# vshiv18/khoice

Measured on AMD Instinct MI355X. Metric: distinct k-mers/sec (k=31, canonical), higher is better.
Workload: dtype u64

## Files before the change

khoice_amd/csrc/kh_engine.cpp:

```cpp
#include <hip/hip_runtime.h>

#include <algorithm>
#include <atomic>
#include <thread>
#include <chrono>
#include <cmath>
#include <memory>
#include <cstdarg>
#include <cstdio>
#include <cstdlib>
#include <cstring>
#include <map>
#include <mutex>
#include <string>
#include <vector>

#include "../../include/khoice_hip.h"
#include "kh_engine.h"
#include "kh_launch.h"
#include "kh_skm_rec.h"

static thread_local std::string g_last_error;

int kh_fail(int code, const char* fmt, ...) {
// ... 1789 lines not shown
    HIPCHK(hipMemcpyAsync(s->dev<u8>(off.ginfo), h_up, up_bytes, hipMemcpyHostToDevice, st));
    c->prof_end();

    KhSkmJob& job = s->job;
    job.seg_tag = by_group ? s->dev<const u8>(off.tags) : nullptr;
    job.segs = s->dev<const KhSeg>(off.segs);
    job.tiles = s->dev<const KhTile>(off.tiles);
    job.reg1 = s->d_reg1.as<uint4>();
    job.reg2 = s->d_reg2.as<uint4>();
    job.cur1 = s->dev<u32>(off.cur1);
    job.cur2 = s->dev<u32>(off.cur2);
    job.inst = s->dev<unsigned long long>(off.inst);
    job.dup = s->dev<unsigned long long>(off.dup);
    job.ginfo = s->dev<const u32>(off.ginfo);
    job.hist = s->dev<unsigned long long>(0);
    job.ctl = s->dev<u32>(off.ctl);
    job.claim = s->dev<u32>(off.claim);
    job.tile_pos = tile_pos;
    job.k = k; job.m = g.m; job.w = g.w; job.nmax = g.nmax;
    job.nslots = g.nslots; job.S = g.S; job.nb1 = g.nb1; job.cap1 = g.cap1; job.cap2 = g.cap2;
    job.nbins = L->nbins; job.abase = L->abase; job.reps = reps; job.nops = by_group ? (u32)ngroups : (u32)nseq;
    job.spill_rec = s->d_spill.as<uint4>();
    job.spill_slot = reinterpret_cast<u32*>(s->d_spill.as<u8>() + (size_t)spill_cap * rec_bytes);
    job.big_list = reinterpret_cast<u32*>(s->d_spill.as<u8>() + (size_t)spill_cap * (rec_bytes + 4));
    job.spill_cap = spill_cap;
    job.big_cap = SkmRun::big_cap;
#ifdef KH_STAMPS
    const u64 nst = std::max<u64>(ntiles, g.nslots);
    TMP_ALLOC(s->d_stamps, c, 128 * nst);
    HIPCHK(hipMemsetAsync(s->d_stamps.b->p, 0, 128 * nst, st));
    kh_debug_set_stamps_skm(s->d_stamps.as<u64>());
#endif
    c->prof_begin(KC_SKM_SCATTER);
    wd.scatter(job, ntiles, st);
    c->prof_end();
#ifdef KH_STAMPS
    report_stamps(c, "skm_scatter (second sub-tile: codes / hashes / minima / slots+count / - / append / barrier / -)", s->d_stamps.b, ntiles);
    HIPCHK(hipMemsetAsync(s->d_stamps.b->p, 0, 128 * nst, st));
    kh_debug_set_stamps_skm(nullptr);
#endif
    c->prof_begin(KC_SKM_REGROUP);
    wd.regroup(job, st);
    c->prof_end();
#ifdef KH_STAMPS
    kh_debug_set_stamps_skm(s->d_stamps.as<u64>());
#ifdef KH_STAMPS_WG
    kh_debug_set_stamps_skm2(s->d_stamps.as<u64>());
#endif
#endif
    s->staged = true;
    return KH_OK;
}
static int exp1_skm(kh_ctx* c, const Exp1In& in, uint64_t* within_hist, uint64_t* across_hist, uint64_t* distinct_per_seq,
                    bool* done, bool by_group = false) {
    *done = false;
    SkmRun s(c);
    KHCHK(skm_prepare(c, in.nseq, in.seqs, in.lens, in.on_device, in.group_of, in.ngroups, in.k, by_group, 0, 0, &s));
    if (!s.staged) return KH_OK;
    const TagLayout& L = s.L;
    const SkmGeometry& g = s.g;
    const KhSkmJob& job = s.job;
    hipStream_t st = c->st;
    KHCHK(timed_launch(c, KC_SKM_UNION, [&] { g.wd->unite(job, in.cs, g.ugrid, st); }));
#if defined(KH_STAMPS) && defined(KH_STAMPS_WG)
    dump_wg_ends(c, s.d_stamps.b, g.ugrid);
    kh_debug_set_stamps_skm(nullptr);
    kh_debug_set_stamps_skm2(nullptr);
#elif defined(KH_STAMPS)
    report_stamps(c, "skm_union (scan barrier / owner / expand / insert / barrier / read-out / barrier / flush)", s.d_stamps.b, g.nslots);
    kh_debug_set_stamps_skm(nullptr);
#endif
    if (getenv("KHOICE_SKM_DEBUG")) {
        std::vector<u32> h1(g.nb1), h2(g.nslots);
        HIPCHK(hipMemcpy2DAsync(h1.data(), 4, job.cur1, 4 * (size_t)KH_SKM_CUR1_STRIDE, 4, g.nb1, hipMemcpyDeviceToHost, st));
        HIPCHK(hipMemcpyAsync(h2.data(), job.cur2, 4 * (size_t)g.nslots, hipMemcpyDeviceToHost, st));
        u32 hc[KH_SKM_CTL_WORDS];
        HIPCHK(hipMemcpyAsync(hc, job.ctl, sizeof hc, hipMemcpyDeviceToHost, st));
        HIPCHK(hipStreamSynchronize(st));
        u64 t1 = 0, t2 = 0;
        u32 m1 = 0, m2 = 0;
        for (u32 v : h1) { t1 += v; m1 = std::max(m1, v); }
        for (u32 v : h2) { t2 += v; m2 = std::max(m2, v); }
        fprintf(stderr, "[skm] k=%d m=%d w=%u nmax=%u positions=%llu records=%llu (%.2f k-mers each) nb1=%u S=%u nslots=%u | "
                        "coarse: mean %.0f max %u cap %u | slot: mean %.1f max %u cap %u | tiles %u x %u | expanded: %u k-mers | errors %u spilled %u overfull slots %u multi-subset slots %u\n",
                in.k, g.m, g.w, g.nmax, (unsigned long long)g.positions, (unsigned long long)t1, (double)g.positions / std::max<u64>(1, t1),
                g.nb1, g.S, g.nslots, (double)t1 / g.nb1, m1, g.cap1, (double)t2 / g.nslots, m2, g.cap2, s.ntiles, job.tile_pos,
                hc[KH_SKM_CTL_EXPANDED], hc[KH_SKM_CTL_ERR], hc[KH_SKM_CTL_SPILLED], hc[KH_SKM_CTL_LISTED], g.two ? 0u : hc[KH_SKM_CTL_MULTI]);
    }
    bool declines = false;
    KHCHK(s.settle(0, [&](u32 nbig) {
        c->stat.big_slots += nbig;
        return timed_launch(c, KC_SKM_BIG, [&] { g.wd->big(job, in.cs, nbig, st); });
    }, &declines));
    if (declines) return KH_OK;
    c->stat.skm_records += s.h_ctl()[KH_SKM_CTL_RECORDS];
    if (!L.by_group) {
        c->stat.bases += s.bases;
        c->stat.builds += L.nseq;
        u64 isum = 0, dsum = 0;
        s.per_text([&](int t, u64 inst, u64 d) {
            isum += inst;
            dsum += d;
            if (distinct_per_seq) distinct_per_seq[t] = d;
        });
        c->stat.kmers += isum;
        c->stat.distinct += dsum;
        c->stat.setop_in += dsum;
    }
    c->stat.setops++;
    std::vector<u64> bins(L.nbins, 0);
    L.add_bins(bins, s.h_hist(), job.reps);
    L.fold(c, bins, within_hist, across_hist, in.hist_len);
    *done = true;
    return KH_OK;
}
static bool skm_exchange_k(int k) { return k >= KH_SKM_MIN_K && k <= KH_SKM_MAX_K; }

static bool skm_exchange_geometry(int k, uint64_t positions_max, int nparts, u32 fan, u64* nslots, double* per_kmer_out,
                                  double eff_parts = 0.0 ) {
    const int m = skm_minimizer_len(k);
    const u32 w = (u32)(k - m + 1);
    const double per_kmer = skm_per_kmer(w);
    const double clump = skm_clump(w, std::max<u32>(1, fan));
    auto region = [&](double mean) { return mean * per_kmer * skm_region_slack(clump, mean) + 128.0; };
    if (eff_parts <= 0.0) eff_parts = (double)nparts;
    double mean = std::min(2600.0 / (0.55 * eff_parts), (1024.0 - 128.0) / (1.7 * per_kmer));
    while (mean > 64.0 && region(mean) > 1008.0) mean *= 0.95;
    if (const char* e = getenv("KHOICE_SKM_EXCHANGE_MEAN")) mean = std::max(16.0, atof(e));
    u64 ns = std::max<u64>((u64)nparts, (u64)((double)std::max<u64>(1, positions_max) / mean) + 1);
    ns = std::min<u64>(ns, (u64)KH_SKM2_MAX_COARSE * KH_SKM_MAX_FINE);
    if (region((double)positions_max / (double)ns) > 1024.0) return false;
    *nslots = ns;
    *per_kmer_out = per_kmer;
    return true;
}
extern "C" int kh_skm_exchange_plan(kh_ctx* c, int k, uint64_t positions_max, uint32_t fan_max, int nparts, uint32_t* nslots,
                                    uint32_t* slots_per_part, uint64_t* part_cap) {
    if (!c || !nslots || !slots_per_part || !part_cap || nparts < 1) return kh_fail(KH_E_ARG, "kh_skm_exchange_plan: bad argument");
    if (!skm_exchange_k(k)) return kh_fail(KH_E_ARG, "the exchange form takes k = %d .. %d", KH_SKM_MIN_K, KH_SKM_MAX_K);
    u64 ns = 0;
    double per_kmer = 0;
    if (!skm_exchange_geometry(k, positions_max, nparts, fan_max, &ns, &per_kmer))
        return kh_fail(KH_E_CAPACITY, "too many k-mers per rank for the exchange form (%llu positions)", (unsigned long long)positions_max);
    *nslots = (u32)ns;
    *slots_per_part = (u32)((ns + nparts - 1) / nparts);
    *part_cap = skm_part_cap(positions_max, per_kmer, nparts);
    return KH_OK;
}

struct SkmPackLocal {
    std::vector<u64> inst;
    u64 dup[32] = {};
    Tmp spill;
    u32 spill_n = 0;
    bool done = false;
};
static int skm_pack_impl(kh_ctx* c, int nseq, const uint8_t* const* seqs, const uint64_t* lens, int on_device,
                         const int* tag_of, int k, uint32_t nslots, int nparts, uint64_t part_cap, void* rec_out,
                         uint32_t* mask_out, uint32_t* count_out, uint32_t* off_out, uint64_t* part_n, SkmPackLocal* loc) {
    if (loc) loc->done = false;
    if (!c || nseq < 0 || (nseq && (!seqs || !lens || !tag_of)) || nparts < 1 || !nslots || !rec_out || !mask_out || !count_out ||
        !off_out || !part_n)
        return kh_fail(KH_E_ARG, "kh_skm_pack: bad argument");
    if (!skm_exchange_k(k)) return kh_fail(KH_E_ARG, "the exchange form takes k = %d .. %d", KH_SKM_MIN_K, KH_SKM_MAX_K);
    int ntags = 0;
    for (int i = 0; i < nseq; ++i) {
        if (tag_of[i] < 0 || tag_of[i] >= 32) return kh_fail(KH_E_ARG, "kh_skm_pack: tag %d outside 0..31", tag_of[i]);
        ntags = std::max(ntags, tag_of[i] + 1);
    }
    HIPCHK(hipSetDevice(c->dev));
// ... 1839 lines not shown
```

khoice_amd/csrc/kh_launch.h:

```cpp
#pragma once
#include <hip/hip_runtime.h>
#include "kh_common.h"

struct KhSeg {
    const u8* seq;
    u64 len;
    u64 npos;
    u64 thist_base;
    u32 nbuckets;
    u32 bucket_base;
    u32 tile_base;
    u32 ntiles;
    u32 nb_virtual;
    u32 b_first;
};
struct KhTile { u32 seg; u32 tile_in_seg; };

struct KhBucketWork {
    u64 lo;
    u64 out_base;
    u32 n;
    u32 nb;
    u32 b;
    u32 gb;
};

struct KhSetView {
    const void* keys;
    const u32* counts;
    u64 n;
    u32 uniform;
    u32 pad;
};

struct KhBoundsJob {
    const KhSetView* sets;
    u64* bounds;
    u64* zero;
    u64 zero_words;
    u32 nsets, nranges;
};

constexpr int KH_SETOP_BATCH = 16;
struct KhSetopJob {
    const KhSetView* sets;
    const u64* bounds;
    void* out_keys;
    u32* out_counts;
    u64* desc;
    u32* ctl;
    unsigned long long* hist;
    u32 nsets;
    u32 nslots;
    u32 slot0, nranges;
};
struct KhSetopBatch { KhSetopJob job[KH_SETOP_BATCH]; };

struct KhGrid {
    u16* off;
    unsigned long long* distinct;
    u32 S;
    u32 nb;
};
constexpr int KH_TAG_MAX_OPS = 64;
constexpr int KH_TAG_MAX_BINS = 255;
struct KhTagJob {
    const void* keys;
    const u64* bstart;
    const u16* off;
    const u32* ginfo;
    unsigned long long* hist;
    u32* ctl;
    u32 nb, S, nops, nbins, abase, ngroups, reps;
    u32 nbv;
    u32 binmul;
    void* out_keys;
    u32* out_counts;
    u64* desc;
    unsigned long long* out_n;
};

#ifndef KH_TUNE_SKM_STAGE
#define KH_TUNE_SKM_STAGE 2048
#endif
constexpr u32 KH_SKM_STAGE = KH_TUNE_SKM_STAGE;
constexpr u32 KH_SKM_MAX_COARSE = 256;
constexpr u32 KH_SKM_MAX_FINE = 512;
constexpr int KH_SKM_MIN_K = 17, KH_SKM_MAX_K = 32;
#ifndef KH_TUNE_SKM_CUR1_STRIDE
#define KH_TUNE_SKM_CUR1_STRIDE 1088
#endif
constexpr u32 KH_SKM_CUR1_STRIDE = KH_TUNE_SKM_CUR1_STRIDE;
enum : u32 {
    KH_SKM_CTL_ERR = 0,
    KH_SKM_CTL_FULLEST = 1,
    KH_SKM_CTL_RECORDS = 2,
    KH_SKM_CTL_EXPANDED = 3,
    KH_SKM_CTL_SPILLED = 5,
    KH_SKM_CTL_LISTED = 6,
    KH_SKM_CTL_MULTI = 7,
    KH_SKM_CTL_WORDS = 8,
};
enum : u32 {
    KH_SKM_XCTL_ERR = 0,
    KH_SKM_XCTL_FULLEST = 1,
    KH_SKM_XCTL_CURSORS = 16,
};
struct KhSkmJob {
    const KhSeg* segs;
    const KhTile* tiles;
    const u8* seg_tag;
    uint4* reg1;
    uint4* reg2;
    u32* cur1;
    u32* cur2;
    unsigned long long* inst;
    unsigned long long* dup;
    const u32* ginfo;
    unsigned long long* hist;
    u32* ctl;
    u32* claim;
    u32 tile_pos;
    int k, m;
    u32 w;
    u32 nmax;
    u32 nslots, S, nb1, cap1, cap2;
    u32 nbins, abase, reps, nops;
    uint4* spill_rec;
    u32* spill_slot;
    u32* big_list;
    u32 spill_cap, big_cap;
};
struct KhSkmCrossJob {
    unsigned long long* bins;
    u32 pmlo, pmhi;
    u32 ngenomes;
    u32 nbins, reps;
    u32 nlisted;
};
struct KhSkmPivotJob {
    KhSkmCrossJob cj;
    u32 pinfo[KH_TAG_MAX_OPS];
};
constexpr int KH_SKM2_MAX_K = 63;
constexpr u32 KH_SKM2_MAX_COARSE = 512;
constexpr u32 KH_SKM2_MAX_FINE = 1024;
struct KhSkmWidth {
    u32 rec_bytes;
    u32 max_coarse, max_fine;
    u32 max_cap2;
    u32 table;
    u32 union_per_cu, cross_per_cu;
    u32 pivot_per_cu;
    u32 cross_round;
    bool (*supports_w)(u32 w);
    void (*scatter)(const KhSkmJob& job, u32 ntiles, hipStream_t st);
    void (*regroup)(const KhSkmJob& job, hipStream_t st);
    void (*unite)(const KhSkmJob& job, u32 cs, u32 grid, hipStream_t st);
    void (*big)(const KhSkmJob& job, u32 cs, u32 nbig, hipStream_t st);
    void (*cross)(const KhSkmJob& job, const KhSkmCrossJob& cj, u32 grid, hipStream_t st);
    void (*pivot)(const KhSkmJob& job, const KhSkmPivotJob& pj, u32 grid, hipStream_t st);
};
const KhSkmWidth& kh_skm_width1();
const KhSkmWidth& kh_skm_width2();
inline const KhSkmWidth& kh_skm_width(bool two) { return two ? kh_skm_width2() : kh_skm_width1(); }
struct KhSkmPackJob {
    const uint4* reg2;
    const u32* cur2;
    uint4* out_rec;
    u32* out_mask;
    u32* part_cursor;
    u32* slot_count;
    u32* slot_off;
    u32* ctl;
    unsigned long long* dup;
    u64 part_cap;
    u32 cap2, nslots, spp;
    u32 nsub;
};
struct KhSkmCompactJob {
// ... 175 lines not shown
```

khoice_amd/csrc/kh_skm.hip:

```cpp
#include <hip/hip_runtime.h>

#include "kh_device.h"
#include "kh_launch.h"

#ifdef KH_STAMPS
__device__ u64* g_skm_stamps = nullptr;
void kh_debug_set_stamps_skm(u64* p) { (void)hipMemcpyToSymbol(HIP_SYMBOL(g_skm_stamps), &p, sizeof p); }
#define SKM_STAMP(idx)                                                                     \
    do {                                                                                   \
        __builtin_amdgcn_sched_barrier(0);                                                 \
        if (threadIdx.x == 0 && g_skm_stamps)                                              \
            g_skm_stamps[((u64)blockIdx.y * gridDim.x + blockIdx.x) * 16 + (idx)] = __builtin_amdgcn_s_memtime(); \
        __builtin_amdgcn_sched_barrier(0);                                                 \
    } while (0)
#else
#define SKM_STAMP(idx) do {} while (0)
#endif

#ifdef KH_MARKS
#define SKM_MARK(name) asm volatile("; ===== MARK " name ::: "memory")
#else
#define SKM_MARK(name) do {} while (0)
#endif
#ifndef KH_TUNE_SKM_SCATTER_PREFETCH
// ... 266 lines not shown
using SkmUnion = SkmUnionGeo<1024, 4096>;
static_assert(SkmUnion::TABLE == 4096, "the slot geometry and its measurements (skm_plan) are the 4096-entry table's");

__device__ __forceinline__ u32 key_hash2(u32 lo, u32 hi) { return (lo ^ hi) * 0x9E3779B1u; }

struct Skm1Consts {
    u32 kml, kmh;
    u32 fsh;
    u32 tsh;
    u32 tsh_sub;
    bool tsh_high;
    __device__ __forceinline__ explicit Skm1Consts(const int k)
        : kml((u32)kh_mask(2 * k)), kmh((u32)(kh_mask(2 * k) >> 32)), fsh(64u - 2u * (u32)k), tsh(2u * (u32)k - 2u),
          tsh_sub(tsh >= 32u ? tsh - 32u : tsh), tsh_high(tsh >= 32u) {}
};
template <int E, class F>
__device__ __forceinline__ void skm1_expand(const uint4 r0, const u32 first, const Skm1Consts& kc, F&& f) {
    const u64 clo = ((u64)r0.y << 32) | r0.x, chi = ((u64)r0.w << 32) | r0.z;
    const u32 sh = 2u * first;
    const u64 lo = sh ? (clo >> sh) | (chi << (64u - sh)) : clo, hi = chi >> sh;
    const u32 xl = (u32)lo & kc.kml, xh = (u32)(lo >> 32) & kc.kmh;
    const u64 fw = kh_revpairs64(((u64)xh << 32) | xl) >> kc.fsh;
    u32 fl = (u32)fw, fh = (u32)(fw >> 32), rl = ~xl & kc.kml, rh = ~xh & kc.kmh;
    const u32 t = (u32)((lo >> kc.tsh) | (hi << (64u - kc.tsh)));
    const u32 tc = ~t;
#pragma unroll
    for (int e = 0; e < E; ++e) {
        if (e) {
            fh = __builtin_amdgcn_alignbit(fh, fl, 30) & kc.kmh;
            fl = ((fl << 2) | ((t >> (2 * e)) & 3u)) & kc.kml;
            rl = __builtin_amdgcn_alignbit(rh, rl, 2);
            rh >>= 2;
            if (kc.tsh_high) rh |= ((tc >> (2 * e)) & 3u) << kc.tsh_sub; else rl |= ((tc >> (2 * e)) & 3u) << kc.tsh_sub;
        }
        const bool fwd = fh < rh || (fh == rh && fl < rl);
        f((u32)e, fwd ? fl : rl, fwd ? fh : rh);
    }
}
struct SkmClaim1 {
    unsigned long long* tkey;
    u32 okey_off;
    unsigned long long empty, K;
    __device__ __forceinline__ u32 operator()(const bool second, const u32 S) const {
        const unsigned long long o2 = atomicCAS(tkey + (second ? okey_off : 0u) + S, empty, K);
        return o2 == empty ? SKM_FRESH : (o2 == K ? SKM_SAME_KEY : SKM_OTHER_KEY);
    }
};

#if defined(KH_STAMPS) && defined(KH_STAMPS_WG)
#define SKM_USTAMP(idx) do {} while (0)
#define SKM_WGSTAMP(idx)                                                                   \
    do {                                                                                   \
        __builtin_amdgcn_sched_barrier(0);                                                 \
        if (threadIdx.x == 0 && g_skm_stamps) {                                            \
            u64* const sp_ = g_skm_stamps + (u64)blockIdx.x * 16;                          \
            sp_[(idx)] = __builtin_amdgcn_s_memtime();                                     \
            sp_[(idx) + 3] = wall_clock64();                                               \
            if ((idx) == 0) {                                                              \
                sp_[1] = __builtin_amdgcn_s_getreg(4 | (31 << 11));                        \
                sp_[2] = __builtin_amdgcn_s_getreg(20 | (31 << 11));                       \
            }                                                                              \
        }                                                                                  \
        __builtin_amdgcn_sched_barrier(0);                                                 \
    } while (0)
#elif defined(KH_STAMPS)
#define SKM_WGSTAMP(idx) do {} while (0)
#define SKM_USTAMP(idx)                                                                    \
    do {                                                                                   \
        __builtin_amdgcn_sched_barrier(0);                                                 \
        if (threadIdx.x == 0 && g_skm_stamps) g_skm_stamps[(u64)slot * 16 + (idx)] = __builtin_amdgcn_s_memtime(); \
        __builtin_amdgcn_sched_barrier(0);                                                 \
    } while (0)
#else
#define SKM_USTAMP(idx) do {} while (0)
#define SKM_WGSTAMP(idx) do {} while (0)
#endif

#ifndef KH_TUNE_SKM_UNION_LEAN
#define KH_TUNE_SKM_UNION_LEAN 1
#endif
#ifndef KH_TUNE_SKM_UNION_KT
#define KH_TUNE_SKM_UNION_KT 1
#endif
template <u32 NT, u32 T, int KT>
__global__ __launch_bounds__(NT, 8) void k_skm_union(const KhSkmJob jb, u32 cs, u32 first_claimed) {
    extern __shared__ __attribute__((aligned(16))) u8 lds_raw[];
    using G = SkmUnionGeo<NT, T>;
    constexpr u32 T2 = G::T2, NW = NT / 64;
    constexpr u32 T2SH = 25;
    constexpr int E = (int)SKM_UE;
    constexpr u64 EMPTY = ~0ull;
    u8* p = lds_raw;
    unsigned long long* tkey = reinterpret_cast<unsigned long long*>(p);   p += (size_t)T * 8;
    u32* tmlo = reinterpret_cast<u32*>(p);                                 p += (size_t)T * 4;
    u32* tmhi = reinterpret_cast<u32*>(p);                                 p += (size_t)T * 4;
    unsigned long long* okey = reinterpret_cast<unsigned long long*>(p);   p += (size_t)T2 * 8;
    u32* omlo = reinterpret_cast<u32*>(p);                                 p += (size_t)T2 * 4;
    u32* omhi = reinterpret_cast<u32*>(p);                                 p += (size_t)T2 * 4;
    uint4* gtab = reinterpret_cast<uint4*>(p);                             p += 1024;
    u32* scratch = reinterpret_cast<u32*>(p);                              p += 128;
    u32* dupc = reinterpret_cast<u32*>(p);                                 p += 256;
    u32* hstripe = reinterpret_cast<u32*>(p);                              p += (size_t)SKM_HSTRIPE_WORDS * 4;
    u16* owner = reinterpret_cast<u16*>(p);                                p += (size_t)G::MAXCH * 2;
    u32* rmask = reinterpret_cast<u32*>(p);
    uint4* stage = reinterpret_cast<uint4*>(tkey);
    u32* dd = reinterpret_cast<u32*>(tkey) + T;
    const u32 tid0 = threadIdx.x, wid = __builtin_amdgcn_readfirstlane(tid0 >> 6);
    u32 tid = tid0, lane = lane_id();
    const u32 nbins = jb.nbins, cap2 = jb.cap2, nslots = jb.nslots;
    const int k = KT ? KT : jb.k;
    const u32 sshift = nbins <= 72u ? 2u : (nbins <= 144u ? 1u : 0u), smask = (1u << sshift) - 1u;
    auto clear_keys = [&]() {
        uint4* k4 = reinterpret_cast<uint4*>(tkey);
        for (u32 i = tid; i < T / 2; i += NT) k4[i] = make_uint4(0xffffffffu, 0xffffffffu, 0xffffffffu, 0xffffffffu);
    };
#if !(defined(KH_ABLATE) && KH_ABLATE == 3)
    constexpr bool MASKS_SELF_CLEAN = true;
#else
    constexpr bool MASKS_SELF_CLEAN = false;
#endif
    auto zero_masks = [&]() {
        for (u32 i = tid; i < T / 2; i += NT) reinterpret_cast<uint4*>(tmlo)[i] = make_uint4(0u, 0u, 0u, 0u);
        if (tid < T2) { omlo[tid] = 0u; omhi[tid] = 0u; }
    };
    auto clear_masks = [&]() {
        if (!MASKS_SELF_CLEAN) zero_masks();
        unsigned long long e0 = EMPTY;
        asm volatile("" : "+v"(e0));
        if (tid < T2) okey[tid] = e0;
    };
    typedef const u32 __attribute__((address_space(4))) * ConstU32;
    const ConstU32 counts = (ConstU32)(unsigned long long)jb.cur2;
    const u32 fit = cap2 < G::MAXREC ? cap2 : G::MAXREC;
    auto count_of = [&](u32 sl) -> u32 {
        const u32 n = sl < nslots ? counts[sl] : 0u;
        return n <= fit ? n : 0u;
    };
    SKM_MARK("init");
    if (MASKS_SELF_CLEAN) zero_masks();
    if (tid < (u32)KH_TAG_MAX_OPS) {
        const u32 g = jb.ginfo[tid], g0 = g & 0xffu, gn = (g >> 8) & 0xffu;
        const u64 gm = gn ? (gn >= 64u ? ~0ull : ((1ull << gn) - 1ull)) << g0 : 0ull;
        gtab[tid] = make_uint4((u32)gm, (u32)(gm >> 32), (g >> 16) << sshift, 0u);
        dupc[tid] = 0;
    }
    if (tid < SKM_HSTRIPE_WORDS) hstripe[tid] = 0;
    if (tid == 0) { scratch[0] = 0; scratch[1] = ~0u; }
    const u32 kml = (u32)kh_mask(2 * k), kmh = (u32)(kh_mask(2 * k) >> 32);
    const u32 fsh = 64u - 2u * (u32)k;
    const u32 tsh = 2u * (u32)k - 2u;
    const bool tsh_high = tsh >= 32u;
    const u32 tsh_sub = tsh_high ? tsh - 32u : tsh;
    auto eval_mask = [&](u32 mlo, u32 mhi) -> bool {
        const u32 lsel = lane & smask;
        u32 ng = 0;
        do {
            const u32 first = mlo ? (u32)__builtin_ctz(mlo) : 32u + (u32)__builtin_ctz(mhi);
            const uint4 g = gtab[first];
            u32 c = (u32)__popc(mlo & g.x) + (u32)__popc(mhi & g.y);
            c = c < cs ? c : cs;
            atomicAdd(&hstripe[g.z + (c << sshift) + lsel], 1u);
            const u32 keep_hi = mlo ? ~0u : mhi - 1u;
            mlo &= ~g.x & (mlo - 1u);
            mhi &= ~g.y & keep_hi;
            ++ng;
        } while (mlo | mhi);
        if (ng == 1u) return true;
        atomicAdd(&hstripe[((jb.abase + (ng < cs ? ng : cs)) << sshift) + lsel], 1u);
        return false;
    };
    u32 st_full = 0, st_exp = 0;
    SkmSlotFeed feed(gridDim.x, nslots, first_claimed);
    u32 slot = blockIdx.x, slot_next = slot + gridDim.x;
    u32 nrec = count_of(slot);
    u32 nrec_next = count_of(slot_next);
    uint4 rr = tid < nrec ? (jb.reg2 + (u64)slot * cap2)[tid] : make_uint4(0, 0, 0, 0);
    SKM_WGSTAMP(0);
    while (slot < nslots) {
        tid = tid0;
        asm volatile("" : "+v"(tid));
        lane = tid & (KH_WAVE - 1u);
        const uint4* __restrict__ reg = jb.reg2 + (u64)slot * cap2;
        if (!nrec && counts[slot] > fit) {
            if (tid0 == 0) {
                const u32 at = atomicAdd(jb.ctl + KH_SKM_CTL_LISTED, 1u);
                if (at < jb.big_cap) jb.big_list[at] = slot;
            }
        }
        u32 nj = 0;
        const u32 tg = SkmRec1::tag(rr.w);
        const u32 rx = rr.x, ry = rr.y, rz = rr.z, rw = rr.w;
        {
            u32 z = 0;
            asm volatile("" : "+v"(z));
            for (u32 i = tid; i < T / 4; i += NT) reinterpret_cast<uint4*>(dd)[i] = make_uint4(z, z, z, z);
        }
        if (tid < nrec) {
            nj = SkmRec1::n(rr.w);
            stage[tid] = rr;
            rmask[tid] = 1u << (tg & 31u);
        }
        SKM_USTAMP(0);
        __syncthreads();
        SKM_USTAMP(1);
        const u32 slot_after = feed.take(scratch + 1);
        const u32 nrec_after = count_of(slot_after);
        const bool draw = feed.wants();
        SKM_MARK("dedup");
        if (__builtin_amdgcn_ballot_w64(nj != 0)) {
            u32 h = rx * 0x9E3779B1u ^ ry * 0x85EBCA77u ^ rz * 0xC2B2AE3Du ^ SkmRec1::content_hash_word(rw) * 0x27D4EB2Fu;
            h ^= h >> 15;
            h *= 0x2C1B3C6Du;
            u32 hp = (u32)(((u64)h * T) >> 32);
            const u32 nch = (nj + (u32)E - 1u) / (u32)E;
            bool pend = nj != 0, won = false;
            while (__builtin_amdgcn_ballot_w64(pend)) {
                if (pend) {
                    const u32 old = atomicCAS(&dd[hp], 0u, tid + 1u);
                    if (old == 0u) {
                        won = true;
                        pend = false;
                    } else {
                        const uint4 o = stage[old - 1u];
                        if (o.x == rx && o.y == ry && o.z == rz && SkmRec1::same_content(o.w, rw)) {
                            const u32 bit = 1u << (tg & 31u);
                            const u32 was = atomicOr(&rmask[old - 1u], bit);
                            if (was & bit) {
                                atomicAdd(&dupc[tg], nj);
                                rmask[tid] = 0u;
                            }
                            pend = false;
                        } else {
                            hp = (hp + 1u) & (T - 1u);
                        }
                    }
                }
            }
            const u32 mine = won ? (nch | (nj << 16)) : 0u;
            const u32 incl = wave_scan_add(mine);
            u32 wbase = 0;
            if (lane == KH_WAVE - 1 && incl) wbase = atomicAdd(&scratch[0], incl);
            wbase = (u32)__builtin_amdgcn_readlane((int)wbase, KH_WAVE - 1);
            if (won) {
                const u32 cstart = (wbase + incl - mine) & 0xffffu;
                if (cstart + nch <= G::MAXCH) {
#pragma unroll
                    for (u32 cc = 0; cc < (1u << SKM_OB); ++cc)
                        if (cc < nch) owner[cstart + cc] = (u16)((tid << SKM_OB) | cc);
                }
            }
        }
        SKM_MARK("dedup_end");
        SKM_USTAMP(2);
        __syncthreads();
        const u32 sc0 = scratch[0];
        if ((sc0 & 0xffffu) > G::MAXCH) {
            if (tid < nrec && rmask[tid] == 0u) {
                const u32 w = stage[tid].w;
                atomicSub(&dupc[SkmRec1::tag(w)], SkmRec1::n(w));
            }
            __syncthreads();
        }
        rr = tid < nrec_next ? (jb.reg2 + (u64)slot_next * cap2)[tid] : make_uint4(0, 0, 0, 0);
        clear_keys();
        clear_masks();
        u32 C = sc0 & 0xffffu, N = sc0 >> 16;
        SKM_USTAMP(3);
        SKM_MARK("after_scan");
        st_full = N > st_full ? N : st_full;
        st_exp += N;
        if (C > G::MAXCH) {
            if (tid == 0) {
                if (jb.big_list) {
                    const u32 at = atomicAdd(jb.ctl + KH_SKM_CTL_LISTED, 1u);
                    if (at < jb.big_cap) jb.big_list[at] = slot;
                } else atomicOr(jb.ctl, KH_ERR_CAPACITY);
            }
            C = 0;
            N = 0;
        }
#if defined(KH_ABLATE) && KH_ABLATE == 1
        C = 0; N = 0;
#endif
        __syncthreads();
        if (tid == 0) scratch[0] = 0;
        SKM_MARK("owner_done");
        SKM_USTAMP(4);
        const u32 R0 = (N + T - 1) / T;
        auto slot_body = [&](auto multi_) __attribute__((always_inline)) {
            constexpr bool MULTI = decltype(multi_)::value;
            const u32 R = MULTI ? R0 : 1u;
            const u32 ctid = tid;
            for (u32 q = 0; q < R; ++q) {
                if (q) { clear_keys(); clear_masks(); __syncthreads(); }
                unsigned long long emptyv = EMPTY;
                asm volatile("" : "+v"(emptyv));
                u32 made[SKM_PASSES][E / 2];
#pragma unroll
                for (u32 ps = 0; ps < SKM_PASSES; ++ps)
#pragma unroll
                    for (int e = 0; e < E / 2; ++e) made[ps][e] = 0u;
                u32 ones = 0;
#pragma unroll
                for (u32 pass = 0; pass < SKM_PASSES; ++pass) {
                    if (pass * NT >= C) break;
                    const u32 c = pass * NT + ctid;
                    u64 kreg[E];
                    u32 slot_[E], act = 0, bits = 0, half = 0;
#pragma unroll
                    for (int e = 0; e < E; ++e) { kreg[e] = EMPTY; slot_[e] = 0; }
                    if (c < C) {
                        const u32 o = owner[c], ri = o >> SKM_OB, first = (o & ((1u << SKM_OB) - 1u)) * (u32)E;
                        const uint4 r0 = reg[ri];
                        bits = rmask[ri];
                        half = SkmRec1::half(r0.w);
                        const u32 left = SkmRec1::n(r0.w) - first;
                        const u32 cnt = left < (u32)E ? left : (u32)E;
                        const u64 clo = ((u64)r0.y << 32) | r0.x, chi = ((u64)r0.w << 32) | r0.z;
                        const u32 sh = 2u * first;
                        const u64 lo = sh ? (clo >> sh) | (chi << (64u - sh)) : clo, hi = chi >> sh;
                        const u32 xl = (u32)lo & kml, xh = (u32)(lo >> 32) & kmh;
                        const u64 fw = kh_revpairs64(((u64)xh << 32) | xl) >> fsh;
                        u32 fl = (u32)fw, fh = (u32)(fw >> 32), rl = ~xl & kml, rh = ~xh & kmh;
                        const u32 t = (u32)((lo >> tsh) | (hi << (64u - tsh)));
                        const u32 tc = ~t;
#pragma unroll
                        for (int e = 0; e < E; ++e) {
                            if (e) {
                                fh = __builtin_amdgcn_alignbit(fh, fl, 30) & kmh;
                                fl = ((fl << 2) | ((t >> (2 * e)) & 3u)) & kml;
                                rl = __builtin_amdgcn_alignbit(rh, rl, 2);
                                rh >>= 2;
                                if (tsh_high) rh |= ((tc >> (2 * e)) & 3u) << tsh_sub; else rl |= ((tc >> (2 * e)) & 3u) << tsh_sub;
                            }
                            const bool fwd = fh < rh || (fh == rh && fl < rl);
                            const u32 cl = fwd ? fl : rl, ch = fwd ? fh : rh;
                            const u32 h = key_hash2(cl, ch);
                            kreg[e] = ((u64)ch << 32) | cl;
                            slot_[e] = (u32)(((u64)h * T) >> 32);
                            if (R != 1 && (u32)e < cnt && (((h >> 4) & 0xffffu) * R) >> 16 == q) act |= 1u << e;
                        }
                        if (R == 1) act = (1u << cnt) - 1u;
                    }
#if defined(KH_ABLATE) && KH_ABLATE == 2
                    if (kreg[0] != 0x1234567ull) act = 0;
#endif
                    SKM_MARK("expanded");
                    if (!__builtin_amdgcn_ballot_w64(act != 0)) continue;
                    u32* const mp = half ? tmhi : tmlo;
                    u32 was[E];
#pragma unroll
                    for (int e = 0; e < E; ++e) was[e] = 0u;
                    u32 mk = 0;
                    for (u32 round = 0; round < (u32)KH_TUNE_SKM_FULL_ROUNDS && __builtin_amdgcn_ballot_w64(act != 0); ++round) {
                        unsigned long long old[E];
#pragma unroll
                        for (int e = 0; e < E; ++e)
                            old[e] = (act & (1u << e)) ? atomicCAS(&tkey[slot_[e]], emptyv, (unsigned long long)kreg[e]) : 0ull;
#pragma unroll
                        for (int e = 0; e < E; ++e) {
                            if (act & (1u << e)) {
                                const bool fresh = old[e] == emptyv;
                                if (fresh || old[e] == kreg[e]) {
                                    was[e] = atomicOr(mp + slot_[e], bits);
                                    act &= ~(1u << e);
                                    if (fresh) mk |= 1u << e;
                                } else {
                                    slot_[e] = (slot_[e] + 1u) & (T - 1u);
                                }
                            }
                        }
                    }
                    SKM_USTAMP(9);
                    SKM_MARK("rounds_done");
                    u32 f16[E];
#pragma unroll
                    for (int e = 0; e < E; ++e) f16[e] = (mk >> e) & 1u ? (0x8000u | slot_[e]) : 0u;
                    while (__builtin_amdgcn_ballot_w64(act != 0)) {
                        const bool have_one = act != 0;
                        const u32 es = have_one ? (u32)__builtin_ctz(act) : 0u;
                        u64 K = 0;
#pragma unroll
                        for (int e = 0; e < E; ++e)
                            if (es == (u32)e) K = kreg[e];
                        const u32 H = key_hash2((u32)K, (u32)(K >> 32));
                        u32 S = ((H ^ (H >> 15)) * 0x85EBCA77u) >> T2SH, probes = 0, level = 1;
                        bool mine = have_one;
                        u32 where = 0;
                        while (__builtin_amdgcn_ballot_w64(mine)) {
                            if (mine) {
                                unsigned long long* kp = level == 1 ? okey : tkey;
                                const unsigned long long o2 = atomicCAS(&kp[S], emptyv, (unsigned long long)K);
                                if (o2 == emptyv || o2 == K) {
                                    u32* mp2 = level == 1 ? (half ? omhi : omlo) : mp;
                                    u32 d = atomicOr(mp2 + S, bits) & bits;
                                    while (d) { atomicAdd(&dupc[half * 32u + (u32)__builtin_ctz(d)], 1u); d &= d - 1u; }
                                    if (o2 == emptyv) where = 0x8000u | (level == 1 ? 0x4000u : 0u) | S;
                                    mine = false;
                                } else {
                                    ++probes;
                                    if (level == 1 && probes >= 8u) {
                                        level = 2; probes = 0;
                                        S = (u32)(((u64)H * T) >> 32) + (u32)KH_TUNE_SKM_FULL_ROUNDS;
                                        S = S & (T - 1u);
                                    } else if (level == 2 && probes >= T) {
                                        atomicOr(jb.ctl, KH_ERR_CAPACITY);
                                        mine = false;
                                    } else {
                                        S = level == 1 ? ((S + 1u) & (T2 - 1u)) : ((S + 1u) & (T - 1u));
                                    }
                                }
                            }
                        }
                        if (have_one) {
                            act &= ~(1u << es);
#pragma unroll
                            for (int e = 0; e < E; ++e)
                                if (es == (u32)e) f16[e] = where;
                        }
                    }
                    SKM_MARK("serial_done");
#pragma unroll
                    for (int e = 0; e < E / 2; ++e) made[pass][e] = f16[2 * e] | (f16[2 * e + 1] << 16);
                    {
                        u32 d = 0;
#pragma unroll
                        for (int e = 0; e < E; ++e) d |= was[e] & bits;
                        if (d) {
#pragma unroll
                            for (int e = 0; e < E; ++e) {
                                u32 de = was[e] & bits;
                                while (de) { atomicAdd(&dupc[half * 32u + (u32)__builtin_ctz(de)], 1u); de &= de - 1u; }
                            }
                        }
                    }
                }
                SKM_MARK("insert_done");
                SKM_USTAMP(5);
                if (draw && q == 0 && tid0 == NT - KH_WAVE) feed.draw(jb.claim, scratch + 1);
                __syncthreads();
                SKM_USTAMP(6);
#pragma unroll
                for (u32 pass = 0; pass < SKM_PASSES; ++pass) {
                    u32 any = 0;
#pragma unroll
                    for (int e = 0; e < E / 2; ++e) any |= made[pass][e];
#if defined(KH_ABLATE) && KH_ABLATE == 3
                    if (any != 0x7654321u) any = 0;
#endif
                    if (!__builtin_amdgcn_ballot_w64(any != 0)) continue;
#pragma unroll
                    for (int e = 0; e < E; ++e) {
                        const u32 f = (made[pass][e >> 1] >> (16 * (e & 1))) & 0xffffu;
                        if (f & 0x8000u) {
                            const u32 at = f & 0x3fffu;
                            const bool second = f & 0x4000u;
                            u32 mlo, mhi;
                            if (MASKS_SELF_CLEAN) {
                                mlo = atomicExch((second ? omlo : tmlo) + at, 0u);
                                mhi = atomicExch((second ? omhi : tmhi) + at, 0u);
                            } else {
                                mlo = (second ? omlo : tmlo)[at];
                                mhi = (second ? omhi : tmhi)[at];
                            }
                            if (eval_mask(mlo, mhi)) ++ones;
                        }
                    }
                }
                if (__builtin_amdgcn_ballot_w64(ones != 0)) {
                    ones = wave_scan_add(ones);
                    if (lane == KH_WAVE - 1) atomicAdd(&hstripe[(jb.abase + 1u) << sshift], ones);
                }
                SKM_MARK("readout_done");
                SKM_USTAMP(7);
                if (q + 1 < R) __syncthreads();
            }
        };
        if (KH_TUNE_SKM_UNION_LEAN && R0 == 1u) {
            slot_body(std::false_type{});
        } else if (__builtin_expect(R0 != 0u, 0)) {
            if (R0 > 1u && tid0 == 0) atomicAdd(jb.ctl + KH_SKM_CTL_MULTI, 1u);
            slot_body(std::true_type{});
        }
        SKM_USTAMP(8);
        if (draw && R0 == 0 && tid0 == NT - KH_WAVE) feed.draw(jb.claim, scratch + 1);
        nrec = nrec_next;
        nrec_next = nrec_after;
        slot = slot_next;
        slot_next = slot_after;
    }
    SKM_WGSTAMP(8);
    __syncthreads();
    tid = tid0;
    lane = tid & (KH_WAVE - 1u);
    unsigned long long* __restrict__ rep = jb.hist + (u64)(blockIdx.x % jb.reps) * nbins;
    for (u32 i = tid; i < nbins; i += NT) {
        u32 v = 0;
        for (u32 j = 0; j <= smask; ++j) v += hstripe[(i << sshift) + j];
        if (v) atomicAdd(&rep[i], (unsigned long long)v);
    }
    if (tid < (u32)KH_TAG_MAX_OPS && dupc[tid]) atomicAdd(&jb.dup[tid], (unsigned long long)dupc[tid]);
    if (tid == 0) {
        if (st_full > T) atomicMax(jb.ctl + KH_SKM_CTL_FULLEST, st_full);
        atomicAdd(jb.ctl + KH_SKM_CTL_EXPANDED, st_exp);
    }
}

constexpr u32 SKM_BIG_T = 4096, SKM_BIG_T2 = 128;
struct SkmBig1 {
    using Rec = SkmRec1;
    using Consts = Skm1Consts;
    using Key = unsigned long long;
    static constexpr u32 T = SKM_BIG_T, T2 = SKM_BIG_T2, KEY_BYTES = 8, BATCH = 256, OB = SKM_OB;
    static constexpr int E = (int)SKM_UE;
    template <class F> static __device__ __forceinline__ void expand(const SkmRecord<1>& r, const u32 first, const Consts& kc, F&& f) {
        skm1_expand<E>(r.v[0], first, kc, [&](const u32 e, const u32 cl, const u32 ch) __attribute__((always_inline)) { f(e, ((u64)ch << 32) | cl); });
    }
    static __device__ __forceinline__ u32 hash(const Key K) { return key_hash2((u32)K, (u32)(K >> 32)); }
    static __device__ __forceinline__ SkmClaim1 claim(u8* kmain, const u32 okey_off, const Key K) {
        return SkmClaim1{reinterpret_cast<unsigned long long*>(kmain), okey_off, ~0ull, K};
    }
};
static_assert(skm_big_lds_bytes<SkmBig1>() == 94720, "k_skm_big<SkmBig1>: the walk's LDS with 288 stripe words and the side-list index");
static_assert(skm_cross_lds_bytes<SkmBig1>(false) == 81280 && skm_cross_lds_bytes<SkmBig1>(true) == 97664, "k_skm_cross<SkmBig1>: direct and listed launch");

static size_t skm_pack_lds_bytes(u32 nt) { return (size_t)nt * 16 + (size_t)nt * 4 * 4 + (size_t)nt * 4 + 64; }

template <u32 NT>
__global__ __launch_bounds__(NT) void k_skm_pack(const KhSkmPackJob jb) {
    extern __shared__ __attribute__((aligned(16))) u8 lds_raw[];
    constexpr u32 T = 4 * NT, TSH = NT == 1024 ? 20u : (NT == 512 ? 21u : 22u);
    static_assert(NT == 1024 || NT == 512 || NT == 256, "table of 4 NT entries, a power of two");
    uint4* stage = reinterpret_cast<uint4*>(lds_raw);
    u32* dd = reinterpret_cast<u32*>(lds_raw + (size_t)NT * 16);
    u32* rmask = dd + T;
    u32* scratch = rmask + NT;
// ... 445 lines not shown
```

Before: 117.2 billion.

## Raise wave priority in union dedup/serial tail and add compacted tail walk

```diff
diff --git a/khoice_amd/csrc/kh_engine.cpp b/khoice_amd/csrc/kh_engine.cpp
--- a/khoice_amd/csrc/kh_engine.cpp
+++ b/khoice_amd/csrc/kh_engine.cpp
@@ -1895,10 +1895,10 @@
         for (u32 v : h1) { t1 += v; m1 = std::max(m1, v); }
         for (u32 v : h2) { t2 += v; m2 = std::max(m2, v); }
         fprintf(stderr, "[skm] k=%d m=%d w=%u nmax=%u positions=%llu records=%llu (%.2f k-mers each) nb1=%u S=%u nslots=%u | "
-                        "coarse: mean %.0f max %u cap %u | slot: mean %.1f max %u cap %u | tiles %u x %u | expanded: %u k-mers | errors %u spilled %u overfull slots %u multi-subset slots %u\n",
+                        "coarse: mean %.0f max %u cap %u | slot: mean %.1f max %u cap %u | tiles %u x %u | expanded: %u k-mers | errors %u spilled %u overfull slots %u multi-subset slots %u tail-wide waves %u\n",
                 in.k, g.m, g.w, g.nmax, (unsigned long long)g.positions, (unsigned long long)t1, (double)g.positions / std::max<u64>(1, t1),
                 g.nb1, g.S, g.nslots, (double)t1 / g.nb1, m1, g.cap1, (double)t2 / g.nslots, m2, g.cap2, s.ntiles, job.tile_pos,
-                hc[KH_SKM_CTL_EXPANDED], hc[KH_SKM_CTL_ERR], hc[KH_SKM_CTL_SPILLED], hc[KH_SKM_CTL_LISTED], g.two ? 0u : hc[KH_SKM_CTL_MULTI]);
+                hc[KH_SKM_CTL_EXPANDED], hc[KH_SKM_CTL_ERR], hc[KH_SKM_CTL_SPILLED], hc[KH_SKM_CTL_LISTED], g.two ? 0u : hc[KH_SKM_CTL_MULTI], g.two ? 0u : hc[KH_SKM_CTL_TAILWIDE]);
     }
     bool declines = false;
     KHCHK(s.settle(0, [&](u32 nbig) {
diff --git a/khoice_amd/csrc/kh_launch.h b/khoice_amd/csrc/kh_launch.h
--- a/khoice_amd/csrc/kh_launch.h
+++ b/khoice_amd/csrc/kh_launch.h
@@ -96,6 +96,7 @@
     KH_SKM_CTL_FULLEST = 1,
     KH_SKM_CTL_RECORDS = 2,
     KH_SKM_CTL_EXPANDED = 3,
+    KH_SKM_CTL_TAILWIDE = 4,
     KH_SKM_CTL_SPILLED = 5,
     KH_SKM_CTL_LISTED = 6,
     KH_SKM_CTL_MULTI = 7,
diff --git a/khoice_amd/csrc/kh_skm.hip b/khoice_amd/csrc/kh_skm.hip
--- a/khoice_amd/csrc/kh_skm.hip
+++ b/khoice_amd/csrc/kh_skm.hip
@@ -372,6 +372,17 @@
 #ifndef KH_TUNE_SKM_UNION_KT
 #define KH_TUNE_SKM_UNION_KT 1
 #endif
+#ifndef KH_TUNE_SKM_UNION_PRIO
+#define KH_TUNE_SKM_UNION_PRIO 1
+#endif
+#ifndef KH_TUNE_SKM_UNION_PRIO_LEVEL
+#define KH_TUNE_SKM_UNION_PRIO_LEVEL 1
+#endif
+#ifndef KH_TUNE_SKM_UNION_COMPACT
+#define KH_TUNE_SKM_UNION_COMPACT 0
+#endif
+#define SKM_UNION_PRIO_UP(bit)   do { if ((KH_TUNE_SKM_UNION_PRIO) & (bit)) __builtin_amdgcn_s_setprio(KH_TUNE_SKM_UNION_PRIO_LEVEL); } while (0)
+#define SKM_UNION_PRIO_DOWN(bit) do { if ((KH_TUNE_SKM_UNION_PRIO) & (bit)) __builtin_amdgcn_s_setprio(0); } while (0)
 template <u32 NT, u32 T, int KT>
 __global__ __launch_bounds__(NT, 8) void k_skm_union(const KhSkmJob jb, u32 cs, u32 first_claimed) {
     extern __shared__ __attribute__((aligned(16))) u8 lds_raw[];
@@ -498,6 +509,7 @@
         const bool draw = feed.wants();
         SKM_MARK("dedup");
         if (__builtin_amdgcn_ballot_w64(nj != 0)) {
+            SKM_UNION_PRIO_UP(1);
             u32 h = rx * 0x9E3779B1u ^ ry * 0x85EBCA77u ^ rz * 0xC2B2AE3Du ^ SkmRec1::content_hash_word(rw) * 0x27D4EB2Fu;
             h ^= h >> 15;
             h *= 0x2C1B3C6Du;
@@ -539,6 +551,7 @@
                         if (cc < nch) owner[cstart + cc] = (u16)((tid << SKM_OB) | cc);
                 }
             }
+            SKM_UNION_PRIO_DOWN(1);
         }
         SKM_MARK("dedup_end");
         SKM_USTAMP(2);
@@ -590,6 +603,11 @@
                 for (u32 ps = 0; ps < SKM_PASSES; ++ps)
 #pragma unroll
                     for (int e = 0; e < E / 2; ++e) made[ps][e] = 0u;
+                constexpr bool COMPACT = !MULTI && KH_TUNE_SKM_UNION_COMPACT != 0 && E == 2;
+                constexpr bool WALKER = COMPACT && KH_TUNE_SKM_UNION_COMPACT == 1;
+                u32 walked[(SKM_PASSES + 1) / 2];
+#pragma unroll
+                for (u32 ps = 0; ps < (SKM_PASSES + 1) / 2; ++ps) walked[ps] = 0u;
                 u32 ones = 0;
 #pragma unroll
                 for (u32 pass = 0; pass < SKM_PASSES; ++pass) {
@@ -642,7 +660,7 @@
 #pragma unroll
                     for (int e = 0; e < E; ++e) was[e] = 0u;
                     u32 mk = 0;
-                    for (u32 round = 0; round < (u32)KH_TUNE_SKM_FULL_ROUNDS && __builtin_amdgcn_ballot_w64(act != 0); ++round) {
+                    auto probe_round = [&]() __attribute__((always_inline)) {
                         unsigned long long old[E];
 #pragma unroll
                         for (int e = 0; e < E; ++e)
@@ -660,36 +678,30 @@
                                 }
                             }
                         }
-                    }
-                    SKM_USTAMP(9);
-                    SKM_MARK("rounds_done");
+                    };
                     u32 f16[E];
-#pragma unroll
-                    for (int e = 0; e < E; ++e) f16[e] = (mk >> e) & 1u ? (0x8000u | slot_[e]) : 0u;
-                    while (__builtin_amdgcn_ballot_w64(act != 0)) {
-                        const bool have_one = act != 0;
-                        const u32 es = have_one ? (u32)__builtin_ctz(act) : 0u;
-                        u64 K = 0;
-#pragma unroll
-                        for (int e = 0; e < E; ++e)
-                            if (es == (u32)e) K = kreg[e];
-                        const u32 H = key_hash2((u32)K, (u32)(K >> 32));
-                        u32 S = ((H ^ (H >> 15)) * 0x85EBCA77u) >> T2SH, probes = 0, level = 1;
-                        bool mine = have_one;
-                        u32 where = 0;
+                    auto chain_home = [&](const u32 H) __attribute__((always_inline)) -> u32 { return ((H ^ (H >> 15)) * 0x85EBCA77u) >> T2SH; };
+                    auto tier_walk = [&](auto from_main_, const unsigned long long K, const u32 H, const u32 kbits, const u32 khalf,
+                                         u32 S, u32 probes, bool mine) __attribute__((always_inline)) -> u32 {
+                        constexpr bool FROM_MAIN = decltype(from_main_)::value;
+                        u32* const kmp = khalf ? tmhi : tmlo;
+                        u32 level = FROM_MAIN ? 0u : 1u, where = 0;
                         while (__builtin_amdgcn_ballot_w64(mine)) {
                             if (mine) {
                                 unsigned long long* kp = level == 1 ? okey : tkey;
-                                const unsigned long long o2 = atomicCAS(&kp[S], emptyv, (unsigned long long)K);
+                                const unsigned long long o2 = atomicCAS(&kp[S], emptyv, K);
                                 if (o2 == emptyv || o2 == K) {
-                                    u32* mp2 = level == 1 ? (half ? omhi : omlo) : mp;
-                                    u32 d = atomicOr(mp2 + S, bits) & bits;
-                                    while (d) { atomicAdd(&dupc[half * 32u + (u32)__builtin_ctz(d)], 1u); d &= d - 1u; }
+                                    u32* mp2 = level == 1 ? (khalf ? omhi : omlo) : kmp;
+                                    u32 d = atomicOr(mp2 + S, kbits) & kbits;
+                                    while (d) { atomicAdd(&dupc[khalf * 32u + (u32)__builtin_ctz(d)], 1u); d &= d - 1u; }
                                     if (o2 == emptyv) where = 0x8000u | (level == 1 ? 0x4000u : 0u) | S;
                                     mine = false;
                                 } else {
                                     ++probes;
-                                    if (level == 1 && probes >= 8u) {
+                                    if (FROM_MAIN && level == 0 && probes >= (u32)KH_TUNE_SKM_FULL_ROUNDS) {
+                                        level = 1; probes = 0;
+                                        S = chain_home(H);
+                                    } else if (level == 1 && probes >= 8u) {
                                         level = 2; probes = 0;
                                         S = (u32)(((u64)H * T) >> 32) + (u32)KH_TUNE_SKM_FULL_ROUNDS;
                                         S = S & (T - 1u);
@@ -702,11 +714,83 @@
                                 }
                             }
                         }
-                        if (have_one) {
-                            act &= ~(1u << es);
+                        return where;
+                    };
+                    auto serial_finish = [&]() __attribute__((always_inline)) {
+                        while (__builtin_amdgcn_ballot_w64(act != 0)) {
+                            const bool have_one = act != 0;
+                            const u32 es = have_one ? (u32)__builtin_ctz(act) : 0u;
+                            u64 K = 0;
 #pragma unroll
                             for (int e = 0; e < E; ++e)
-                                if (es == (u32)e) f16[e] = where;
+                                if (es == (u32)e) K = kreg[e];
+                            const u32 H = key_hash2((u32)K, (u32)(K >> 32));
+                            const u32 where = tier_walk(std::false_type{}, (unsigned long long)K, H, bits, half, chain_home(H), 0u, have_one);
+                            if (have_one) {
+                                act &= ~(1u << es);
+#pragma unroll
+                                for (int e = 0; e < E; ++e)
+                                    if (es == (u32)e) f16[e] = where;
+                            }
+                        }
+                    };
+                    if (!COMPACT) {
+                        for (u32 round = 0; round < (u32)KH_TUNE_SKM_FULL_ROUNDS && __builtin_amdgcn_ballot_w64(act != 0); ++round) probe_round();
+                        SKM_USTAMP(9);
+                        SKM_MARK("rounds_done");
+#pragma unroll
+                        for (int e = 0; e < E; ++e) f16[e] = (mk >> e) & 1u ? (0x8000u | slot_[e]) : 0u;
+                        if (((KH_TUNE_SKM_UNION_PRIO) & 2) && !MULTI) {
+                            if (__builtin_amdgcn_ballot_w64(act != 0)) {
+                                SKM_UNION_PRIO_UP(2);
+                                serial_finish();
+                                SKM_UNION_PRIO_DOWN(2);
+                            }
+                        } else {
+                            serial_finish();
+                        }
+                    } else {
+                        probe_round();
+                        SKM_USTAMP(9);
+                        SKM_MARK("rounds_done");
+#pragma unroll
+                        for (int e = 0; e < E; ++e) f16[e] = (mk >> e) & 1u ? (0x8000u | slot_[e]) : 0u;
+                        const u64 b0 = __builtin_amdgcn_ballot_w64((act & 1u) != 0), b1 = __builtin_amdgcn_ballot_w64((act & 2u) != 0);
+                        const u32 L0 = (u32)__popcll(b0), L = L0 + (u32)__popcll(b1);
+                        if (L > KH_WAVE) {
+                            if (lane == 0) atomicAdd(jb.ctl + KH_SKM_CTL_TAILWIDE, 1u);
+                            for (u32 round = 1; round < (u32)KH_TUNE_SKM_FULL_ROUNDS && __builtin_amdgcn_ballot_w64(act != 0); ++round) probe_round();
+#pragma unroll
+                            for (int e = 0; e < E; ++e) f16[e] = (mk >> e) & 1u ? (0x8000u | slot_[e]) : 0u;
+                            serial_finish();
+                        } else if (L) {
+                            SKM_UNION_PRIO_UP(2);
+                            const u32 n0 = __builtin_amdgcn_mbcnt_hi((u32)(b0 >> 32), __builtin_amdgcn_mbcnt_lo((u32)b0, 0u));
+                            const u32 n1 = __builtin_amdgcn_mbcnt_hi((u32)(b1 >> 32), __builtin_amdgcn_mbcnt_lo((u32)b1, 0u));
+                            const u32 d0 = ((act & 1u) ? n0 : L0 + (lane - n0)) << 2;
+                            const u32 d1 = ((act & 2u) ? L0 + n1 : L + (lane - n1)) << 2;
+                            const bool sel0 = lane < L0;
+                            auto packed = [&](const u32 v0, const u32 v1) __attribute__((always_inline)) -> u32 {
+                                const u32 r0 = (u32)__builtin_amdgcn_ds_permute((int)d0, (int)v0);
+                                const u32 r1 = (u32)__builtin_amdgcn_ds_permute((int)d1, (int)v1);
+                                return sel0 ? r0 : r1;
+                            };
+                            const u32 wkl = packed((u32)kreg[0], (u32)kreg[1]), wkh = packed((u32)(kreg[0] >> 32), (u32)(kreg[1] >> 32));
+                            const u32 wph = packed(slot_[0] | (half << 16), slot_[1] | (half << 16));
+                            const u32 wbits = packed(bits, bits);
+                            const unsigned long long K = ((unsigned long long)wkh << 32) | wkl;
+                            static_assert(!COMPACT || KH_TUNE_SKM_FULL_ROUNDS >= 2, "the packed walk enters the main table's rounds at probe 2");
+                            const u32 where = tier_walk(std::true_type{}, K, key_hash2(wkl, wkh), wbits, wph >> 16, wph & 0xffffu, 1u, lane < L);
+                            if (WALKER) {
+                                walked[pass >> 1] |= where << (16u * (pass & 1u));
+                            } else {
+                                const u32 w0 = (u32)__builtin_amdgcn_ds_bpermute((int)d0, (int)where);
+                                const u32 w1 = (u32)__builtin_amdgcn_ds_bpermute((int)d1, (int)where);
+                                if (act & 1u) f16[0] = w0;
+                                if (act & 2u) f16[1] = w1;
+                            }
+                            act = 0;
+                            SKM_UNION_PRIO_DOWN(2);
                         }
                     }
                     SKM_MARK("serial_done");
@@ -727,7 +811,13 @@
                 }
                 SKM_MARK("insert_done");
                 SKM_USTAMP(5);
-                if (draw && q == 0 && tid0 == NT - KH_WAVE) feed.draw(jb.claim, scratch + 1);
+                if ((KH_TUNE_SKM_UNION_PRIO) & 4) {
+                    if (draw && q == 0 && wid == NW - 1u) {
+                        SKM_UNION_PRIO_UP(4);
+                        if (tid0 == NT - KH_WAVE) feed.draw(jb.claim, scratch + 1);
+                        SKM_UNION_PRIO_DOWN(4);
+                    }
+                } else if (draw && q == 0 && tid0 == NT - KH_WAVE) feed.draw(jb.claim, scratch + 1);
                 __syncthreads();
                 SKM_USTAMP(6);
 #pragma unroll
@@ -735,13 +825,15 @@
                     u32 any = 0;
 #pragma unroll
                     for (int e = 0; e < E / 2; ++e) any |= made[pass][e];
+                    const u32 walked_f = WALKER ? (walked[pass >> 1] >> (16u * (pass & 1u))) & 0xffffu : 0u;
+                    any |= walked_f;
 #if defined(KH_ABLATE) && KH_ABLATE == 3
                     if (any != 0x7654321u) any = 0;
 #endif
                     if (!__builtin_amdgcn_ballot_w64(any != 0)) continue;
 #pragma unroll
-                    for (int e = 0; e < E; ++e) {
-                        const u32 f = (made[pass][e >> 1] >> (16 * (e & 1))) & 0xffffu;
+                    for (int e = 0; e < E + (WALKER ? 1 : 0); ++e) {
+                        const u32 f = e < E ? (made[pass][(e < E ? e : 0) >> 1] >> (16 * (e & 1))) & 0xffffu : walked_f;
                         if (f & 0x8000u) {
                             const u32 at = f & 0x3fffu;
                             const bool second = f & 0x4000u;
```

New measurement: 119.1 billion (median of 6 runs). 1.6% higher.
